# MoayedHajiAli/ElasticDiffusion-official

Measured on AMD Instinct MI355X. Metric: images/sec at 50 steps (SDXL 2048x1024), higher is better.
Workload: dtype fp16

## Files before the change

elasticdiffusion_official_amd/csrc/attention_kernels.hip:

```cpp
#include <hip/hip_runtime.h>
#include <stdint.h>

#include "elastic_hip.h"

namespace {

constexpr int D = 64;
constexpr int QB = 128;
constexpr int KT = 64;
constexpr int K_LD = 72;
constexpr int V_LD_TR = 96;
constexpr int V_LD_T = 68;

typedef float f32x16 __attribute__((ext_vector_type(16)));
typedef float f32x8 __attribute__((ext_vector_type(8)));
typedef short s16x4 __attribute__((ext_vector_type(4)));
typedef short s16x8 __attribute__((ext_vector_type(8)));
typedef __bf16 bf16x8 __attribute__((ext_vector_type(8)));
typedef _Float16 f16x8 __attribute__((ext_vector_type(8)));

struct alignas(16) Vec16 { uint32_t w[4]; };
struct alignas(8) Vec8 { uint32_t w[2]; };

struct BF {
// ... 174 lines not shown
#pragma unroll
      for (int kb = 0; kb < 2; ++kb)
#pragma unroll
        for (int r = 0; r < 16; ++r) {
          const float e = __builtin_amdgcn_exp2f(__builtin_fmaf(s[qn][kb][r], sl, -mb));
          s[qn][kb][r] = e;
          psum += e;
        }
      l_run[qn] = __builtin_fmaf(l_run[qn], alpha, psum);
#pragma unroll
      for (int i = 0; i < 16; ++i) {
        oacc[qn][0][i] *= alpha;
        oacc[qn][1][i] *= alpha;
      }
    }

#pragma unroll
    for (int st = 0; st < 4; ++st) {
      typename T::v8 pf[QN];
#pragma unroll
      for (int qn = 0; qn < QN; ++qn) {
        f32x8 pv;
#pragma unroll
        for (int j = 0; j < 8; ++j) pv[j] = s[qn][st >> 1][8 * (st & 1) + j];
        pf[qn] = T::pack(pv);
      }
#pragma unroll
      for (int db = 0; db < 2; ++db) {
        Vec16 vf;
        if (TR) {
          const int row = 16 * st + 4 * hi + ((lane & 15) >> 2);
          const int col = 32 * db + 16 * ((lane >> 4) & 1) + 4 * (lane & 3);
          typedef s16x4 __attribute__((address_space(3))) * lds_s16x4_ptr;
          const s16x4 lo = __builtin_amdgcn_ds_read_tr16_b64_v4i16((lds_s16x4_ptr)(&sm.v[buf][row * V_LD_TR + col]));
          const s16x4 hi4 = __builtin_amdgcn_ds_read_tr16_b64_v4i16((lds_s16x4_ptr)(&sm.v[buf][(row + 8) * V_LD_TR + col]));
          const s16x8 both = __builtin_shufflevector(lo, hi4, 0, 1, 2, 3, 4, 5, 6, 7);
          vf = __builtin_bit_cast(Vec16, both);
        } else {
          const uint16_t* vrow = &sm.v[buf][(32 * db + ln) * V_LD_T + 16 * st + 4 * hi];
          const Vec8 lo = *reinterpret_cast<const Vec8*>(vrow);
          const Vec8 hi8 = *reinterpret_cast<const Vec8*>(vrow + 8);
          vf.w[0] = lo.w[0], vf.w[1] = lo.w[1], vf.w[2] = hi8.w[0], vf.w[3] = hi8.w[1];
        }
#pragma unroll
        for (int qn = 0; qn < QN; ++qn) oacc[qn][db] = T::mfma(as_v8<typename T::v8>(vf), pf[qn], oacc[qn][db]);
      }
    }

    if (t + 1 < n_tiles) write_lds(buf ^ 1);
    __syncthreads();
  }

#pragma unroll
  for (int qn = 0; qn < QN; ++qn) {
    const float l_tot = l_run[qn] + __shfl_xor(l_run[qn], 32, 64);
    const float inv = 1.0f / l_tot;
    if (q_row[qn] < p.Nq) {
      uint16_t* orow = og + (int64_t)q_row[qn] * p.o_sn;
#pragma unroll
      for (int db = 0; db < 2; ++db)
#pragma unroll
        for (int g = 0; g < 4; ++g) {
          f32x8 tmp;
#pragma unroll
          for (int e = 0; e < 4; ++e) tmp[e] = oacc[qn][db][4 * g + e] * inv, tmp[4 + e] = 0.f;
          const Vec16 packed = __builtin_bit_cast(Vec16, T::pack(tmp));
          Vec8 out8 = {{packed.w[0], packed.w[1]}};
          *reinterpret_cast<Vec8*>(orow + 32 * db + 8 * g + 4 * hi) = out8;
        }
    }
  }
}


constexpr float RESCALE_LOG2 = 6.0f;
constexpr float RESCALE_SUM_MAX = 64.0f;

template <int NK>
struct SmemPipe {
  uint16_t k[NK][KT * K_LD];
  uint16_t v[3][KT * V_LD_TR];
};

template <typename T>
__device__ __forceinline__ void qk_tile(const uint16_t* kt, int ln, int hi, const typename T::v8 (&qf)[4], f32x16 (&s)[2]) {
#pragma unroll
  for (int i = 0; i < 16; ++i) s[0][i] = s[1][i] = 0.f;
#pragma unroll
  for (int ks = 0; ks < 4; ++ks)
#pragma unroll
    for (int kb = 0; kb < 2; ++kb) {
      const Vec16 kf = *reinterpret_cast<const Vec16*>(&kt[(32 * kb + ln) * K_LD + 16 * ks + 8 * hi]);
      s[kb] = T::mfma(as_v8<typename T::v8>(kf), qf[ks], s[kb]);
    }
}

__device__ __forceinline__ Vec16 v_frag_tr(const uint16_t* vt, int lane, int hi, int st, int db) {
  const int row = 16 * st + 4 * hi + ((lane & 15) >> 2);
  const int col = 32 * db + 16 * ((lane >> 4) & 1) + 4 * (lane & 3);
  typedef s16x4 __attribute__((address_space(3))) * lds_s16x4_ptr;
  const s16x4 lo = __builtin_amdgcn_ds_read_tr16_b64_v4i16((lds_s16x4_ptr)(&vt[row * V_LD_TR + col]));
  const s16x4 hi4 = __builtin_amdgcn_ds_read_tr16_b64_v4i16((lds_s16x4_ptr)(&vt[(row + 8) * V_LD_TR + col]));
  return __builtin_bit_cast(Vec16, __builtin_shufflevector(lo, hi4, 0, 1, 2, 3, 4, 5, 6, 7));
}

template <typename T>
__device__ __forceinline__ void pv_tile(const uint16_t* vt, int lane, int hi, const typename T::v8 (&pf)[4], f32x16 (&o)[2]) {
#pragma unroll
  for (int st = 0; st < 4; ++st)
#pragma unroll
    for (int db = 0; db < 2; ++db)
      o[db] = T::mfma(as_v8<typename T::v8>(v_frag_tr(vt, lane, hi, st, db)), pf[st], o[db]);
}

typedef __amdgpu_buffer_rsrc_t BufRsrc;
typedef uint32_t u32x4 __attribute__((ext_vector_type(4)));
__device__ __forceinline__ BufRsrc make_rsrc(const void* base, int64_t bytes) {
  const uint64_t a = (uint64_t)base;
  const uint32_t lo = __builtin_amdgcn_readfirstlane((int)(uint32_t)a), hi = __builtin_amdgcn_readfirstlane((int)(uint32_t)(a >> 32));
  const uint32_t n = __builtin_amdgcn_readfirstlane((int)(uint32_t)(bytes > 0xffffffffll ? 0xffffffffll : (bytes < 0 ? 0 : bytes)));
  return __builtin_amdgcn_make_buffer_rsrc((void*)(((uint64_t)hi << 32) | lo),  0, (int)n, 0x00020000);
}
__device__ __forceinline__ Vec16 buf_load16(BufRsrc rs, uint32_t voff, uint32_t soff) {
  const u32x4 v = __builtin_bit_cast(u32x4, __builtin_amdgcn_raw_buffer_load_b128(rs, voff, soff, 0));
  Vec16 o = {{v[0], v[1], v[2], v[3]}};
  return o;
}


template <typename T, int NDB = 2>
__device__ __forceinline__ void store_o_row(uint16_t* orow, const f32x16 (&o)[NDB], float inv, int hi, bool valid, int dh = 64) {
#pragma unroll
  for (int db = 0; db < NDB; ++db) {
    uint32_t part[4][2];
#pragma unroll
    for (int g = 0; g < 4; ++g) {
      f32x8 tmp;
#pragma unroll
      for (int e = 0; e < 4; ++e) tmp[e] = o[db][4 * g + e] * inv, tmp[4 + e] = 0.f;
      const Vec16 packed = __builtin_bit_cast(Vec16, T::pack(tmp));
      part[g][0] = packed.w[0], part[g][1] = packed.w[1];
    }
#pragma unroll
    for (int gp = 0; gp < 2; ++gp) {
      const int ge = 2 * gp, go = 2 * gp + 1;
      const uint32_t r0 = __shfl_xor(hi ? part[ge][0] : part[go][0], 32, 64);
      const uint32_t r1 = __shfl_xor(hi ? part[ge][1] : part[go][1], 32, 64);
      Vec16 out;
      if (hi) out = Vec16{{r0, r1, part[go][0], part[go][1]}};
      else out = Vec16{{part[ge][0], part[ge][1], r0, r1}};
      const int d0 = 32 * db + 8 * (hi ? go : ge);
      if (valid && d0 < dh) *reinterpret_cast<Vec16*>(orow + d0) = out;
    }
  }
}

struct True { static constexpr bool value = true; };
struct False { static constexpr bool value = false; };

struct SoftmaxRun {
  float mb;
  float l;
  float mx;
  float use;
  float alpha;
  float psum;
};

template <typename T>
__device__ __forceinline__ void softmax_slice(int i, f32x16 (&s)[2], float sl, SoftmaxRun& r, typename T::v8 (&pf)[4]) {
  if (i < 2) {
    float mx = (i == 0) ? -INFINITY : r.mx;
#pragma unroll
    for (int j = 0; j < 16; j += 2) mx = fmaxf(fmaxf(mx, s[i][j]), s[i][j + 1]);
    r.mx = mx;
    asm volatile("" : "+v"(r.mx));
  } else if (i == 2) {
    const float mx = fmaxf(r.mx, __shfl_xor(r.mx, 32, 64));
    const float mbn = mx * sl;
    r.use = (mbn - r.mb > RESCALE_LOG2) ? mbn : r.mb;
    r.alpha = __builtin_amdgcn_exp2f(r.mb - r.use);
    r.mb = r.use;
    r.psum = 0.f;
    asm volatile("" : "+v"(r.use), "+v"(r.alpha));
  } else if (i < 15) {
    const int g = (i - 3) / 3, w = (i - 3) % 3;
    const int f0 = 8 * g + 3 * w, n = (w == 2) ? 2 : 3;
#pragma unroll
    for (int j = 0; j < n; ++j) {
      const int f = f0 + j;
      const float e = __builtin_amdgcn_exp2f(__builtin_fmaf(s[f >> 4][f & 15], sl, -r.use));
      s[f >> 4][f & 15] = e;
      r.psum += e;
    }
    asm volatile("" : "+v"(r.psum));
    if (w == 2) {
      f32x8 pv;
#pragma unroll
      for (int j = 0; j < 8; ++j) pv[j] = s[g >> 1][8 * (g & 1) + j];
      pf[g] = T::pack(pv);
      asm volatile("" : "+v"(pf[g]));
    }
  } else {
    r.l = __builtin_fmaf(r.l, r.alpha, r.psum);
  }
}

template <typename T, bool EXP2>
__device__ __forceinline__ void softmax_slice_lazy(int i, f32x16 (&s)[2], float sl, SoftmaxRun& r, typename T::v8 (&pf)[4]) {
  if (i == 0) r.psum = 0.f;
#pragma unroll
  for (int j = 0; j < 2; ++j) {
    const int f = 2 * i + j;
    const float e = EXP2 ? __builtin_amdgcn_exp2f(s[f >> 4][f & 15])
                         : __builtin_amdgcn_exp2f(__builtin_fmaf(s[f >> 4][f & 15], sl, -r.mb));
    s[f >> 4][f & 15] = e;
    r.psum += e;
  }
  asm volatile("" : "+v"(r.psum));
  if ((i & 3) == 3) {
    const int g = i >> 2;
    f32x8 pv;
#pragma unroll
    for (int j = 0; j < 8; ++j) pv[j] = s[g >> 1][8 * (g & 1) + j];
    pf[g] = T::pack(pv);
    asm volatile("" : "+v"(pf[g]));
  }
}

template <typename T>
__device__ __forceinline__ void resoftmax_tile(const uint16_t* kt, int ln, int hi, const typename T::v8 (&qf)[4],
                                               f32x16 (&s)[2], float sl, SoftmaxRun& r, typename T::v8 (&pf)[4]) {
  qk_tile<T>(kt, ln, hi, qf, s);
  float mx = s[0][0];
#pragma unroll
  for (int j = 1; j < 16; ++j) mx = fmaxf(mx, s[0][j]);
#pragma unroll
  for (int j = 0; j < 16; ++j) mx = fmaxf(mx, s[1][j]);
  mx = fmaxf(mx, __shfl_xor(mx, 32, 64));
  const float use = fmaxf(r.mb, mx * sl);
  r.alpha = __builtin_amdgcn_exp2f(r.mb - use);
  r.mb = use;
  float psum = 0.f;
#pragma unroll
  for (int g = 0; g < 4; ++g) {
    f32x8 pv;
#pragma unroll
    for (int j = 0; j < 8; ++j) {
      const int f = 8 * g + j;
      pv[j] = __builtin_amdgcn_exp2f(__builtin_fmaf(s[f >> 4][f & 15], sl, -use));
      psum += pv[j];
    }
    pf[g] = T::pack(pv);
  }
  r.psum = psum;
}

template <typename T, bool HAS_PV, bool HAS_NEXT, bool LAZY, bool EXP2, int DEPTH, class Filler>
__device__ __forceinline__ void pipe_region(Filler&& filler, const uint16_t* k_next, const uint16_t* v_prev, int lane, int ln, int hi,
                                            const typename T::v8 (&qf)[4], f32x16 (&s_cur)[2], f32x16 (&s_next)[2],
                                            const typename T::v8 (&p_prev)[4], typename T::v8 (&p_cur)[4],
                                            f32x16 (&o)[2], float sl, SoftmaxRun& run, const f32x16& negm) {
  constexpr int NQK = HAS_NEXT ? 8 : 0, N = NQK + (HAS_PV ? 8 : 0);
  auto fetch = [&](int i) -> Vec16 {
    if (i < NQK) return *reinterpret_cast<const Vec16*>(&k_next[(32 * (i & 1) + ln) * K_LD + 16 * (i >> 1) + 8 * hi]);
    const int j = i - NQK;
    return v_frag_tr(v_prev, lane, hi, j >> 1, j & 1);
  };
  if (HAS_NEXT && !EXP2) {
#pragma unroll
    for (int i = 0; i < 16; ++i) s_next[0][i] = s_next[1][i] = 0.f;
  }
  Vec16 ring[DEPTH + 1];
#pragma unroll
  for (int r = 0; r <= DEPTH; ++r) ring[r] = Vec16{{0u, 0u, 0u, 0u}};
#pragma unroll
  for (int r = 0; r < DEPTH; ++r)
    if (r < N) ring[r] = fetch(r);
#pragma unroll
  for (int i = 0; i < 16; ++i) {
    if (i < N) {
      if (i + DEPTH < N) ring[(i + DEPTH) % (DEPTH + 1)] = fetch(i + DEPTH);
      const Vec16 a_cur = ring[i % (DEPTH + 1)];
      if (i < NQK) {
        if (EXP2 && i < 2) s_next[i & 1] = T::mfma(as_v8<typename T::v8>(a_cur), qf[0], negm);
        else s_next[i & 1] = T::mfma(as_v8<typename T::v8>(a_cur), qf[i >> 1], s_next[i & 1]);
        asm volatile("" : "+v"(s_next[i & 1]));
      } else {
        const int j = i - NQK;
        o[j & 1] = T::mfma(as_v8<typename T::v8>(a_cur), p_prev[j >> 1], o[j & 1]);
        asm volatile("" : "+v"(o[j & 1]));
      }
    }
    if (LAZY) softmax_slice_lazy<T, EXP2>(i, s_cur, sl, run, p_cur);
    else softmax_slice<T>(i, s_cur, sl, run, p_cur);
    filler(i);
    __builtin_amdgcn_sched_barrier(0);
  }
}

template <typename T, bool LAZY, bool EXP2 = false, int DEPTH = 1, int WAVES = 4>
__global__ void __launch_bounds__(64 * WAVES, 2)
k_flash_attn_pipe(const Params p) {
  static_assert(LAZY || !EXP2, "the exponent-domain variant is built on the lazy-maximum loop");
  static_assert(WAVES == 4 || WAVES == 8, "4 or 8 waves per workgroup");
  constexpr int NK = LAZY ? 3 : 2;
  constexpr int NST = 8 / WAVES;
  __shared__ SmemPipe<NK> sm;
  const int tid = threadIdx.x;
  const int lane = tid & 63, wave = tid >> 6;
  const int ln = lane & 31, hi = lane >> 5;
  int bh, qblk;
  {
    const int id = blockIdx.x, per = 8 * p.nqb, grp = id / per, r = id - grp * per;
    if ((grp + 1) * 8 <= p.BH) {
      bh = grp * 8 + (r & 7);
      qblk = r >> 3;
    } else {
      bh = grp * 8 + r / p.nqb;
      qblk = r % p.nqb;
    }
  }
  const int b = bh / p.H, h = bh - b * p.H;
  const uint16_t* qg = p.q + b * p.q_sb + h * D;
  const uint16_t* kg = p.k + b * p.k_sb + h * D;
  const uint16_t* vg = p.v + b * p.v_sb + h * D;
  uint16_t* og = p.o + b * p.o_sb + h * D;

  const int q_row = qblk * (32 * WAVES) + wave * 32 + ln;
  typename T::v8 qf[4];
#pragma unroll
  for (int ks = 0; ks < 4; ++ks) qf[ks] = as_v8<typename T::v8>(load_row16(qg, p.q_sn, q_row, p.Nq, 16 * ks + 8 * hi));

  const BufRsrc k_rs = make_rsrc(kg, ((int64_t)(p.Nk - 1) * p.k_sn + D) * 2);
  const BufRsrc v_rs = make_rsrc(vg, ((int64_t)(p.Nk - 1) * p.v_sn + D) * 2);
  const int st_row = tid >> 3, st_col = (tid & 7) * 8;
  const uint32_t k_off = (uint32_t)(((int64_t)st_row * p.k_sn + st_col) * 2), k_half = (uint32_t)(32 * p.k_sn * 2);
  const uint32_t v_off = (uint32_t)(((int64_t)st_row * p.v_sn + st_col) * 2), v_half = (uint32_t)(32 * p.v_sn * 2);
  Vec16 kreg[NST], vreg[NST];
  auto load_k = [&](int t) {
    const uint32_t base = k_off + (uint32_t)t * 2u * k_half;
#pragma unroll
    for (int i = 0; i < NST; ++i) kreg[i] = buf_load16(k_rs, base + i * k_half, 0);
  };
  auto load_v = [&](int t) {
    const uint32_t base = v_off + (uint32_t)t * 2u * v_half;
#pragma unroll
    for (int i = 0; i < NST; ++i) vreg[i] = buf_load16(v_rs, base + i * v_half, 0);
  };
  auto write_k = [&](int buf) {
// ... 75 lines not shown
    }
    const int tmp = vb_prev;
    vb_prev = vb_cur, vb_cur = vb_next, vb_next = tmp;
    const int ktmp = kb_cur;
    kb_cur = kb_next, kb_next = kb_write, kb_write = NK == 3 ? ktmp : kb_cur;
    __syncthreads();
  };

  if (n_full > 0) {
    qk_tile<T>(sm.k[0], ln, hi, qf, sA);
    if (EXP2) {
      float mx = sA[0][0];
#pragma unroll
      for (int j = 1; j < 16; ++j) mx = fmaxf(mx, sA[0][j]);
#pragma unroll
      for (int j = 0; j < 16; ++j) mx = fmaxf(mx, sA[1][j]);
      mx = fmaxf(mx, __shfl_xor(mx, 32, 64));
      run.mb = mx;
#pragma unroll
      for (int i = 0; i < 16; ++i) sA[0][i] -= mx, sA[1][i] -= mx, negm[i] = -mx;
      asm volatile("" : "+v"(negm));
    }
    __syncthreads();
    if (n_full == 1) {
      iter(False{}, False{}, 0, sA, sB, pB, pA);
    } else {
      iter(False{}, True{}, 0, sA, sB, pB, pA);
      int t = 1;
      for (; t + 2 < n_full; t += 2) {
        iter(True{}, True{}, t, sB, sA, pA, pB);
        iter(True{}, True{}, t + 1, sA, sB, pB, pA);
      }
      if (n_full - t == 2) {
        iter(True{}, True{}, t, sB, sA, pA, pB);
        iter(True{}, False{}, t + 1, sA, sB, pB, pA);
      } else {
        iter(True{}, False{}, t, sB, sA, pA, pB);
      }
    }
    if ((n_full - 1) & 1) pv_tile<T>(sm.v[vb_prev], lane, hi, pB, oacc);
    else pv_tile<T>(sm.v[vb_prev], lane, hi, pA, oacc);
  }

  if (n_tiles > n_full) {
    f32x16 s[2];
    qk_tile<T>(sm.k[kb_cur], ln, hi, qf, s);
#pragma unroll
    for (int kb = 0; kb < 2; ++kb)
#pragma unroll
      for (int r = 0; r < 16; ++r)
        if (n_full * KT + 32 * kb + 8 * (r >> 2) + 4 * hi + (r & 3) >= p.Nk) s[kb][r] = -INFINITY;
    float mx = s[0][0];
#pragma unroll
    for (int r = 1; r < 16; ++r) mx = fmaxf(mx, s[0][r]);
#pragma unroll
    for (int r = 0; r < 16; ++r) mx = fmaxf(mx, s[1][r]);
    mx = fmaxf(mx, __shfl_xor(mx, 32, 64));
    const float use = fmaxf(run.mb, mx * sl);
    const float alpha = __builtin_amdgcn_exp2f(run.mb - use);
    float psum = 0.f;
#pragma unroll
    for (int kb = 0; kb < 2; ++kb)
#pragma unroll
      for (int r = 0; r < 16; ++r) {
        const float e = __builtin_amdgcn_exp2f(__builtin_fmaf(s[kb][r], sl, -use));
        s[kb][r] = e;
        psum += e;
      }
    run.l = __builtin_fmaf(run.l, alpha, psum);
#pragma unroll
    for (int i = 0; i < 16; ++i) {
      oacc[0][i] *= alpha;
      oacc[1][i] *= alpha;
    }
    typename T::v8 pf[4];
#pragma unroll
    for (int st = 0; st < 4; ++st) {
      f32x8 pv;
#pragma unroll
      for (int j = 0; j < 8; ++j) pv[j] = s[st >> 1][8 * (st & 1) + j];
      pf[st] = T::pack(pv);
    }
    pv_tile<T>(sm.v[vb_cur], lane, hi, pf, oacc);
  }

  const float l_tot = run.l + __shfl_xor(run.l, 32, 64);
  const float inv = 1.0f / l_tot;
  store_o_row<T>(og + (int64_t)q_row * p.o_sn, oacc, inv, hi, q_row < p.Nq);
}

constexpr int SK_QBLOCKS = 4;

template <int NKB>
struct SmemSmall {
  uint16_t k[32 * NKB * K_LD];
  uint16_t v[32 * NKB * V_LD_TR];
};

template <typename T, int NKB>
__global__ void __launch_bounds__(256, 2)
k_flash_attn_smallkv(const Params p) {
  __shared__ SmemSmall<NKB> sm;
  const int tid = threadIdx.x;
  const int lane = tid & 63, wave = tid >> 6;
  const int ln = lane & 31, hi = lane >> 5;
  const int nqg = p.nqb;
  const int bh = blockIdx.x / nqg, qgrp = blockIdx.x - bh * nqg;
  const int b = bh / p.H, h = bh - b * p.H;
  const uint16_t* qg = p.q + b * p.q_sb + h * D;
  const uint16_t* kg = p.k + b * p.k_sb + h * D;
  const uint16_t* vg = p.v + b * p.v_sb + h * D;
  uint16_t* og = p.o + b * p.o_sb + h * D;

  for (int idx = tid; idx < 32 * NKB * 8; idx += 256) {
    const int row = idx >> 3, col = (idx & 7) * 8;
    *reinterpret_cast<Vec16*>(&sm.k[row * K_LD + col]) = load_row16(kg, p.k_sn, row, p.Nk, col);
    *reinterpret_cast<Vec16*>(&sm.v[row * V_LD_TR + col]) = load_row16(vg, p.v_sn, row, p.Nk, col);
  }
  __syncthreads();
  const float sl = p.scale_log2e;

  for (int qb = 0; qb < SK_QBLOCKS; ++qb) {
    const int q_row = (qgrp * SK_QBLOCKS + qb) * QB + wave * 32 + ln;
    if ((qgrp * SK_QBLOCKS + qb) * QB + wave * 32 >= p.Nq) break;
    typename T::v8 qf[4];
#pragma unroll
    for (int ks = 0; ks < 4; ++ks) qf[ks] = as_v8<typename T::v8>(load_row16(qg, p.q_sn, q_row, p.Nq, 16 * ks + 8 * hi));
    f32x16 s[NKB];
#pragma unroll
    for (int kb = 0; kb < NKB; ++kb)
#pragma unroll
      for (int i = 0; i < 16; ++i) s[kb][i] = 0.f;
#pragma unroll
    for (int ks = 0; ks < 4; ++ks)
#pragma unroll
      for (int kb = 0; kb < NKB; ++kb) {
        const Vec16 kf = *reinterpret_cast<const Vec16*>(&sm.k[(32 * kb + ln) * K_LD + 16 * ks + 8 * hi]);
        s[kb] = T::mfma(as_v8<typename T::v8>(kf), qf[ks], s[kb]);
      }
    float mx = -INFINITY;
#pragma unroll
    for (int kb = 0; kb < NKB; ++kb)
#pragma unroll
      for (int r = 0; r < 16; ++r) {
        if (32 * kb + 8 * (r >> 2) + 4 * hi + (r & 3) >= p.Nk) s[kb][r] = -INFINITY;
        mx = fmaxf(mx, s[kb][r]);
      }
    mx = fmaxf(mx, __shfl_xor(mx, 32, 64));
    const float mb = mx * sl;
    float psum = 0.f;
#pragma unroll
    for (int kb = 0; kb < NKB; ++kb)
#pragma unroll
      for (int r = 0; r < 16; ++r) {
        const float e = __builtin_amdgcn_exp2f(__builtin_fmaf(s[kb][r], sl, -mb));
        s[kb][r] = e;
        psum += e;
      }
    psum += __shfl_xor(psum, 32, 64);
    const float inv = 1.0f / psum;
    f32x16 o[2];
#pragma unroll
    for (int i = 0; i < 16; ++i) o[0][i] = o[1][i] = 0.f;
#pragma unroll
    for (int st = 0; st < 2 * NKB; ++st) {
      f32x8 pv;
// ... 128 lines not shown
#pragma unroll
    for (int r = 0; r < 16; ++r) mx = fmaxf(mx, s[1][r]);
    mx = fmaxf(mx, __shfl_xor(mx, 32, 64));
    const float m_new = fmaxf(m_run, mx);
    const float mb = m_new * sl;
    const float alpha = __builtin_amdgcn_exp2f(__builtin_fmaf(m_run, sl, -mb));
    m_run = m_new;
    float psum = 0.f;
#pragma unroll
    for (int kb = 0; kb < 2; ++kb)
#pragma unroll
      for (int r = 0; r < 16; ++r) {
        const float e = __builtin_amdgcn_exp2f(__builtin_fmaf(s[kb][r], sl, -mb));
        s[kb][r] = e;
        psum += e;
      }
    l_run = __builtin_fmaf(l_run, alpha, psum);
#pragma unroll
    for (int db = 0; db < G::NDB; ++db)
#pragma unroll
      for (int i = 0; i < 16; ++i) oacc[db][i] *= alpha;

#pragma unroll
    for (int st = 0; st < 4; ++st) {
      f32x8 pv;
#pragma unroll
      for (int j = 0; j < 8; ++j) pv[j] = s[st >> 1][8 * (st & 1) + j];
      const typename T::v8 pf = T::pack(pv);
#pragma unroll
      for (int db = 0; db < G::NDB; ++db) {
        const int row = 16 * st + 4 * hi + ((lane & 15) >> 2);
        const int col = 32 * db + 16 * ((lane >> 4) & 1) + 4 * (lane & 3);
        typedef s16x4 __attribute__((address_space(3))) * lds_s16x4_ptr;
        const s16x4 lo = __builtin_amdgcn_ds_read_tr16_b64_v4i16((lds_s16x4_ptr)(&sm.v[buf][row * G::VLD + col]));
        const s16x4 hi4 = __builtin_amdgcn_ds_read_tr16_b64_v4i16((lds_s16x4_ptr)(&sm.v[buf][(row + 8) * G::VLD + col]));
        const Vec16 vf = __builtin_bit_cast(Vec16, __builtin_shufflevector(lo, hi4, 0, 1, 2, 3, 4, 5, 6, 7));
        oacc[db] = T::mfma(as_v8<typename T::v8>(vf), pf, oacc[db]);
      }
    }
    if (t + 1 < n_tiles) write_lds(buf ^ 1);
    __syncthreads();
  }

  const float l_tot = l_run + __shfl_xor(l_run, 32, 64);
  const float inv = 1.0f / l_tot;
  store_o_row<T, G::NDB>(og + (int64_t)q_row * p.o_sn, oacc, inv, hi, q_row < p.Nq, DH);
}

}

extern "C" {

int ed_flash_attention(const void* q, const void* k, const void* v, void* out, int dtype, int B, int H, int Nq, int Nk,
                       int head_dim, int64_t q_sb, int64_t q_sn, int64_t k_sb, int64_t k_sn, int64_t v_sb, int64_t v_sn,
                       int64_t o_sb, int64_t o_sn, float scale, int v_path, void* stream) {
  if (B == 0 || H == 0 || Nq == 0) return 0;
  if (Nk <= 0) return (int)hipErrorInvalidValue;
  if (head_dim != D) {
    if (head_dim != 40 && head_dim != 80 && head_dim != 160) return (int)hipErrorInvalidValue;
    if (dtype != ED_BF16 && dtype != ED_F16) return (int)hipErrorInvalidValue;
    if ((((uintptr_t)q | (uintptr_t)k | (uintptr_t)v) & 15u) || ((uintptr_t)out & 7u)) return (int)hipErrorInvalidValue;
    if ((q_sb | q_sn | k_sb | k_sn | v_sb | v_sn) % 8 || (o_sb | o_sn) % 4) return (int)hipErrorInvalidValue;
    Params p;
    p.q = (const uint16_t*)q, p.k = (const uint16_t*)k, p.v = (const uint16_t*)v, p.o = (uint16_t*)out;
    p.Nq = Nq, p.Nk = Nk, p.H = H, p.BH = B * H, p.nqb = (Nq + QB - 1) / QB;
    p.q_sb = q_sb, p.q_sn = q_sn, p.k_sb = k_sb, p.k_sn = k_sn, p.v_sb = v_sb, p.v_sn = v_sn, p.o_sb = o_sb, p.o_sn = o_sn;
    p.scale_log2e = scale * 1.44269504088896340736f;
    const int64_t nb = (int64_t)p.BH * p.nqb;
    if (nb > 0x7fffffff) return (int)hipErrorInvalidValue;
    const dim3 grid((unsigned)nb), block(256);
    hipStream_t st = (hipStream_t)stream;
#define ED_FG(DHV)                                                                      \
  if (dtype == ED_BF16) k_flash_attn_gen<BF, DHV><<<grid, block, 0, st>>>(p);           \
  else k_flash_attn_gen<HF, DHV><<<grid, block, 0, st>>>(p);
    if (head_dim == 40) { ED_FG(40) } else if (head_dim == 80) { ED_FG(80) } else { ED_FG(160) }
#undef ED_FG
    return (int)hipGetLastError();
  }
  if ((((uintptr_t)q | (uintptr_t)k | (uintptr_t)v) & 15u) || ((uintptr_t)out & 7u)) return (int)hipErrorInvalidValue;
  if ((q_sb | q_sn | k_sb | k_sn | v_sb | v_sn) % 8 || (o_sb | o_sn) % 4) return (int)hipErrorInvalidValue;
  Params p;
  p.q = (const uint16_t*)q, p.k = (const uint16_t*)k, p.v = (const uint16_t*)v, p.o = (uint16_t*)out;
  hipStream_t st = (hipStream_t)stream;
  if ((v_path >= 4 && v_path <= 10)) {
    if (v_path == 8 && Nk > 160) return (int)hipErrorInvalidValue;
    if ((v_path == 6 || v_path == 7 || v_path == 9 || v_path == 10) && Nk < 64) return (int)hipErrorInvalidValue;
    if (v_path != 8 && ((int64_t)(Nk + 2 * KT) * (k_sn > v_sn ? k_sn : v_sn) * 2 >= 0x7fffffffll)) return (int)hipErrorInvalidValue;
    const int rows_per_wg = v_path == 8 ? QB * SK_QBLOCKS : (v_path >= 9 ? 2 * QB : QB);
    p.Nq = Nq, p.Nk = Nk, p.H = H, p.BH = B * H, p.nqb = (Nq + rows_per_wg - 1) / rows_per_wg;
    p.q_sb = q_sb, p.q_sn = q_sn, p.k_sb = k_sb, p.k_sn = k_sn, p.v_sb = v_sb, p.v_sn = v_sn, p.o_sb = o_sb, p.o_sn = o_sn;
    p.scale_log2e = scale * 1.44269504088896340736f;
    const int64_t nb = (int64_t)p.BH * p.nqb;
    if (nb > 0x7fffffff) return (int)hipErrorInvalidValue;
    const dim3 grid((unsigned)nb), block(256);
    if (dtype != ED_BF16 && dtype != ED_F16) return (int)hipErrorInvalidValue;
    if (v_path == 4) {
      if (dtype == ED_BF16) k_flash_attn_pipe<BF, false><<<grid, block, 0, st>>>(p);
      else k_flash_attn_pipe<HF, false><<<grid, block, 0, st>>>(p);
    } else if (v_path == 5) {
      if (dtype == ED_BF16) k_flash_attn_pipe<BF, true><<<grid, block, 0, st>>>(p);
      else k_flash_attn_pipe<HF, true><<<grid, block, 0, st>>>(p);
    } else if (v_path == 6) {
      if (dtype == ED_BF16) k_flash_attn_pipe<BF, true, true><<<grid, block, 0, st>>>(p);
      else k_flash_attn_pipe<HF, true, true><<<grid, block, 0, st>>>(p);
    } else if (v_path == 7) {
      if (dtype == ED_BF16) k_flash_attn_pipe<BF, false, false, 3><<<grid, block, 0, st>>>(p);
      else k_flash_attn_pipe<HF, false, false, 3><<<grid, block, 0, st>>>(p);
    } else if (v_path == 9) {
      if (dtype == ED_BF16) k_flash_attn_pipe<BF, false, false, 1, 8><<<grid, dim3(512), 0, st>>>(p);
      else k_flash_attn_pipe<HF, false, false, 1, 8><<<grid, dim3(512), 0, st>>>(p);
    } else if (v_path == 10) {
      if (dtype == ED_BF16) k_flash_attn_pipe<BF, true, false, 1, 8><<<grid, dim3(512), 0, st>>>(p);
      else k_flash_attn_pipe<HF, true, false, 1, 8><<<grid, dim3(512), 0, st>>>(p);
    } else if (Nk <= 64) {
      if (dtype == ED_BF16) k_flash_attn_smallkv<BF, 2><<<grid, block, 0, st>>>(p);
      else k_flash_attn_smallkv<HF, 2><<<grid, block, 0, st>>>(p);
    } else if (Nk <= 96) {
      if (dtype == ED_BF16) k_flash_attn_smallkv<BF, 3><<<grid, block, 0, st>>>(p);
      else k_flash_attn_smallkv<HF, 3><<<grid, block, 0, st>>>(p);
    } else {
      if (dtype == ED_BF16) k_flash_attn_smallkv<BF, 5><<<grid, block, 0, st>>>(p);
      else k_flash_attn_smallkv<HF, 5><<<grid, block, 0, st>>>(p);
    }
    return (int)hipGetLastError();
  }
  const int qn = (v_path & 2) ? 2 : 1;
  p.Nq = Nq, p.Nk = Nk, p.H = H, p.BH = B * H, p.nqb = (Nq + QB * qn - 1) / (QB * qn);
  p.q_sb = q_sb, p.q_sn = q_sn, p.k_sb = k_sb, p.k_sn = k_sn, p.v_sb = v_sb, p.v_sn = v_sn, p.o_sb = o_sb, p.o_sn = o_sn;
  p.scale_log2e = scale * 1.44269504088896340736f;
  const int64_t blocks = (int64_t)p.BH * p.nqb;
  if (blocks > 0x7fffffff) return (int)hipErrorInvalidValue;
  const dim3 grid((unsigned)blocks), block(256);
#define ED_FA(T)                                                                 \
  if (v_path == 0) k_flash_attn_fwd<T, true, 1><<<grid, block, 0, st>>>(p);      \
  else if (v_path == 1) k_flash_attn_fwd<T, false, 1><<<grid, block, 0, st>>>(p); \
  else if (v_path == 2) k_flash_attn_fwd<T, true, 2><<<grid, block, 0, st>>>(p);  \
  else if (v_path == 3) k_flash_attn_fwd<T, false, 2><<<grid, block, 0, st>>>(p); \
  else return (int)hipErrorInvalidValue;
  if (dtype == ED_BF16) {
    ED_FA(BF)
  } else if (dtype == ED_F16) {
    ED_FA(HF)
  } else {
    return (int)hipErrorInvalidValue;
  }
#undef ED_FA
  return (int)hipGetLastError();
}

}
```

elasticdiffusion_official_amd/ops.py:

```python
import torch

from . import _hip

ED_F32, ED_F16, ED_BF16 = 0, 1, 2
_DTYPE = {torch.float32: ED_F32, torch.float16: ED_F16, torch.bfloat16: ED_BF16}


_LAUNCH = {"device": None}


def _stream_of(t):
    if _LAUNCH["device"] is None:
        _LAUNCH["device"] = t.device
    return _stream()


def _stream():
    dev = _LAUNCH["device"]
    if dev is None:
        raise RuntimeError("internal: _stream() before any device tensor argument")
    return torch.cuda.current_stream(dev).cuda_stream


class KernelTimer:
# ... 903 lines not shown
    if not (isinstance(a, torch.Tensor) and a.is_cuda and a.dim() == 4 and a.dtype == torch.float16):
        _reject("conv3x3_f32out_s2: a must be an fp16 [B,C,H,W] tensor on the MI355X; no CPU fallback")
    B, C3, Hi, Wi = a.shape
    N = w.shape[0]
    cl = torch.channels_last
    if tuple(w.shape) != (N, C3, 3, 3) or w.dtype != torch.float16 or not conv3x3_f32out_s2_ok(B, Hi, Wi, C3, N):
        _reject(f"conv3x3_f32out_s2: unsupported shape a {tuple(a.shape)} w {tuple(w.shape)}")
    if not a.is_contiguous(memory_format=cl) or not w.is_contiguous(memory_format=cl):
        _reject("conv3x3_f32out_s2: a and w must be channels_last")
    H, W = Hi // 2, Wi // 2
    out = torch.empty((B, N, H, W), dtype=torch.float32, device=a.device, memory_format=cl)
    TIMER.note_work("ed_conv3x3_nhwc_f32out_s2", flops=2.0 * B * H * W * 9 * C3 * N, nbytes=2.0 * (B * Hi * Wi * C3 + 9 * C3 * N) + 4.0 * B * H * W * N)
    _call("ed_conv3x3_nhwc_f32out_s2", a.data_ptr(), w.data_ptr(), _opt(bias, torch.float32, "bias"), out.data_ptr(), _DTYPE[torch.float16],
          B, H, W, C3, N, float(out_scale), None if act_absmax is None else act_absmax.data_ptr(), _stream_of(a))
    return out


def softmax_rows_(x, scale=1.0):
    cols = x.shape[-1]
    if cols % 4 and x.numel() != cols:
        _reject("softmax_rows_: cols must be a multiple of 4")
    TIMER.note_work("ed_softmax_rows", nbytes=3.0 * x.numel() * 4)
    _call("ed_softmax_rows", _dev(x, torch.float32, "x"), x.numel() // cols, cols, float(scale), _stream())
    return x


VAE_ATTENTION_CHUNK_BYTES = 1 << 30


def vae_attention(q, k, v):
    B, N, C = q.shape
    scale = C ** -0.5
    rows = max(64, min(N, VAE_ATTENTION_CHUNK_BYTES // (4 * N * B) // 64 * 64)) if N > 256 else N
    kt = k.transpose(1, 2)
    if rows >= N:
        return torch.bmm(softmax_rows_(torch.bmm(q, kt), scale), v)
    out = torch.empty_like(q)
    for a in range(0, N, rows):
        s = torch.bmm(q[:, a:a + rows], kt)
        out[:, a:a + rows] = torch.bmm(softmax_rows_(s, scale), v)
    return out


FLASH_V_PATH = None
FLASH_HEAD_DIMS = (40, 64, 80, 160)
FLASH_EXP2 = False
_ENV_VARIANT = __import__("os").environ.get("ED_FLASH_VARIANT")
LOG2E = 1.4426950408889634


def _pipe_fits(Nk, row_stride):
    return Nk >= 128 and (Nk + 128) * row_stride * 2 < 2 ** 31


def flash_prescale(Nq, Nk, row_stride, scale=0.125):
    if FLASH_V_PATH is not None:
        want = int(FLASH_V_PATH)
    elif _ENV_VARIANT is not None:
        want = -1 if _ENV_VARIANT == "legacy" else int(_ENV_VARIANT)
    else:
        want = 6 if FLASH_EXP2 else -1
    return scale * LOG2E if (want == 6 and _pipe_fits(Nk, row_stride)) else None


def _flash_variant(B, heads, Nq, Nk, k=None, v=None, prescaled=False):
    fits = k is None or _pipe_fits(Nk, max(k.stride(1), v.stride(1)))
    if prescaled:
        if not (Nk >= 128 and fits):
            _reject("flash_attention: exponent-domain q needs the pipelined kernel (Nk >= 128, 32-bit K / V offsets)")
        return 6
    if FLASH_V_PATH is not None and int(FLASH_V_PATH) != 6:
        return int(FLASH_V_PATH)
    legacy = 2 if (Nq >= 2048 and Nk >= 1024 and B * heads * (Nq // 256) >= 1024) else 0
    if _ENV_VARIANT == "legacy":
        return legacy
    if _ENV_VARIANT is not None and int(_ENV_VARIANT) != 6:
        want = int(_ENV_VARIANT)
        if want in (4, 5, 7, 9, 10):
            return want if (Nk >= 128 and fits) else (8 if Nk <= 96 else legacy)
        return want if (want != 8 or Nk <= SMALLKV_MAX_KEYS) else legacy
    if Nk <= 96 or _stream_two_chunks(Nq, Nk):
        return 8
    if Nk >= 128 and fits:
        return FLASH_DEFAULT_PIPE
    return legacy


SMALLKV_MAX_KEYS = 160


def _stream_two_chunks(Nq, Nk):
    return 128 <= Nk <= SMALLKV_MAX_KEYS and Nq >= 4096


FLASH_DEFAULT_PIPE = 5


def flash_attention(q, k, v, heads, v_path=None, prescaled=False):
    B, Nq, HD = q.shape
    Nk = k.shape[1]
    hd = HD // heads
    if HD != heads * hd or hd not in FLASH_HEAD_DIMS or k.shape != (B, Nk, HD) or v.shape != (B, Nk, HD):
        _reject(f"flash_attention: head_dim must be one of {FLASH_HEAD_DIMS} and shapes consistent (q {tuple(q.shape)}, "
                f"k {tuple(k.shape)}, v {tuple(v.shape)}, heads {heads})")
    if hd != 64 and (prescaled or v_path is not None):
        _reject("flash_attention: kernel variants exist for head_dim 64 only")
    for t, name in ((q, "q"), (k, "k"), (v, "v")):
        if not t.is_cuda or t.dtype != q.dtype or t.stride(2) != 1:
            _reject(f"flash_attention: {name} must be a 16-bit tensor on the MI355X with unit last stride; no CPU fallback")
        if _LAUNCH["device"] is None:
            _LAUNCH["device"] = t.device
        elif _LAUNCH["device"] != t.device:
            _reject(f"flash_attention: {name} lives on {t.device}, q on {_LAUNCH['device']}")
    if v_path is not None and (int(v_path) == 6) != bool(prescaled):
        _reject("flash_attention: v_path 6 takes exponent-domain q (prescaled=True) and nothing else does")
    out = torch.empty(B, Nq, HD, dtype=q.dtype, device=q.device)
    TIMER.note_work("ed_flash_attention", flops=4.0 * B * heads * Nq * Nk * hd,
                    nbytes=2.0 * q.element_size() * HD * B * (Nq + Nk))
    variant = 0 if hd != 64 else (_flash_variant(B, heads, Nq, Nk, k, v, prescaled) if v_path is None else int(v_path))
    _call("ed_flash_attention", q.data_ptr(), k.data_ptr(), v.data_ptr(), out.data_ptr(), _code(q, "q"), B, heads, Nq, Nk,
          hd, q.stride(0), q.stride(1), k.stride(0), k.stride(1), v.stride(0), v.stride(1), out.stride(0), out.stride(1),
          hd ** -0.5, variant, _stream())
    return out


CANNY_MAX_DIM = 8192


def _canny_dims(t, name, channels):
    if t.dim() == 2 and 1 in channels:
        H, W, C = t.shape[0], t.shape[1], 1
    elif t.dim() == 3 and t.shape[2] in channels:
        H, W, C = t.shape
    else:
        _reject(f"{name} must be uint8 [H,W,C] with C in {sorted(channels)}{' or [H,W]' if 1 in channels else ''}, got {tuple(t.shape)}")
    if not (1 <= H <= CANNY_MAX_DIM and 1 <= W <= CANNY_MAX_DIM):
        _reject(f"{name}: H and W must be in 1..{CANNY_MAX_DIM}, got {H} x {W}")
    return H, W, C


def _canny_threshold(v, name):
    import math
    if not math.isfinite(v):
        _reject(f"canny: {name} threshold must be finite, got {v}")
    return max(-2 ** 31, min(2 ** 31 - 1, int(math.floor(v))))


def canny_map(img, low=100, high=200):
    p_img = _dev(img, torch.uint8, "img")
    H, W, C = _canny_dims(img, "img", (1, 3))
    lo, hi = _canny_threshold(low, "low"), _canny_threshold(high, "high")
    cmap = torch.empty((H, W), dtype=torch.uint8, device=img.device)
    TIMER.note_work("ed_canny_map", nbytes=float(H * W * (C + 1)))
    _call("ed_canny_map", p_img, H, W, C, lo, hi, _dev(cmap, torch.uint8, "map"), _stream())
    return cmap


def canny_hysteresis(cmap):
    import ctypes
    p_map = _dev(cmap, torch.uint8, "map")
    H, W, _ = _canny_dims(cmap, "map", (1,))
    if cmap.dim() != 2:
        _reject(f"map must be [H,W], got {tuple(cmap.shape)}")
    if torch.cuda.is_current_stream_capturing():
        _reject("canny_hysteresis reads a device flag between passes and cannot be captured into a graph")
    ws = torch.empty(_hip.lib().ed_canny_workspace(H, W, 1) // 4, dtype=torch.int32, device=cmap.device)
    passes = ctypes.c_int32(0)
    TIMER.note_work("ed_canny_hysteresis", nbytes=float(H * W))
    _call("ed_canny_hysteresis", p_map, H, W, _dev(ws, torch.int32, "workspace"), ctypes.addressof(passes), _stream())
    return cmap, int(passes.value)


def canny_edges(cmap, out="u8"):
    if out not in ("u8", "cond"):
        raise ValueError(f"out must be 'u8' or 'cond', got {out!r}")
    p_map = _dev(cmap, torch.uint8, "map")
    H, W, _ = _canny_dims(cmap, "map", (1,))
# ... 354 lines not shown
```

Before: 0.1036.

## Add DMA-to-LDS flash attention kernel with swizzled LDS layout for SDXL self-attention shapes

Adds a new flash attention kernel that loads K/V tiles straight from global memory into LDS with buffer_load ... lds. This bypasses the register round trip and the padded staging copies. LDS tiles use an unpadded XOR-swizzled layout to avoid bank conflicts, and the QK/PV fragment readers gain a swizzle-aware path. The dispatcher routes a fixed allowlist of self-attention shapes (B, Nk, heads) to this kernel. The inline-asm m0/waitcnt handling and the shape allowlist add fragility.

```diff
diff --git a/elasticdiffusion_official_amd/csrc/attention_kernels.hip b/elasticdiffusion_official_amd/csrc/attention_kernels.hip
--- a/elasticdiffusion_official_amd/csrc/attention_kernels.hip
+++ b/elasticdiffusion_official_amd/csrc/attention_kernels.hip
@@ -280,7 +280,19 @@
   uint16_t v[3][KT * V_LD_TR];
 };
 
-template <typename T>
+__device__ __forceinline__ constexpr int swz(int row) { return ((row & 2) << 1) | ((row >> 2) & 3); }
+__device__ __forceinline__ int swz_k_lane(int ln, int hi) { return ln * D + ((hi ^ swz(ln)) << 3); }
+__device__ __forceinline__ int swz_v_lane(int lane, int hi) {
+  const int row = 4 * hi + ((lane & 15) >> 2), col = 16 * ((lane >> 4) & 1) + 4 * (lane & 3);
+  return row * D + ((((col >> 3) ^ swz(row)) << 3) | (col & 7));
+}
+template <bool SWZ>
+__device__ __forceinline__ int k_elem(int kb, int ln, int ks, int hi) {
+  if constexpr (SWZ) return 32 * kb * D + (ln ^ (ks << 4));
+  else return (32 * kb + ln) * K_LD + 16 * ks + 8 * hi;
+}
+
+template <typename T, bool SWZ = false>
 __device__ __forceinline__ void qk_tile(const uint16_t* kt, int ln, int hi, const typename T::v8 (&qf)[4], f32x16 (&s)[2]) {
 #pragma unroll
   for (int i = 0; i < 16; ++i) s[0][i] = s[1][i] = 0.f;
@@ -288,27 +300,33 @@
   for (int ks = 0; ks < 4; ++ks)
 #pragma unroll
     for (int kb = 0; kb < 2; ++kb) {
-      const Vec16 kf = *reinterpret_cast<const Vec16*>(&kt[(32 * kb + ln) * K_LD + 16 * ks + 8 * hi]);
+      const Vec16 kf = *reinterpret_cast<const Vec16*>(&kt[k_elem<SWZ>(kb, ln, ks, hi)]);
       s[kb] = T::mfma(as_v8<typename T::v8>(kf), qf[ks], s[kb]);
     }
 }
 
+template <bool SWZ = false>
 __device__ __forceinline__ Vec16 v_frag_tr(const uint16_t* vt, int lane, int hi, int st, int db) {
+  typedef s16x4 __attribute__((address_space(3))) * lds_s16x4_ptr;
+  if constexpr (SWZ) {
+    const s16x4 lo = __builtin_amdgcn_ds_read_tr16_b64_v4i16((lds_s16x4_ptr)(&vt[16 * st * D + (lane ^ (db << 5))]));
+    const s16x4 hi4 = __builtin_amdgcn_ds_read_tr16_b64_v4i16((lds_s16x4_ptr)(&vt[(16 * st + 8) * D + (lane ^ (db << 5) ^ 16)]));
+    return __builtin_bit_cast(Vec16, __builtin_shufflevector(lo, hi4, 0, 1, 2, 3, 4, 5, 6, 7));
+  }
   const int row = 16 * st + 4 * hi + ((lane & 15) >> 2);
   const int col = 32 * db + 16 * ((lane >> 4) & 1) + 4 * (lane & 3);
-  typedef s16x4 __attribute__((address_space(3))) * lds_s16x4_ptr;
   const s16x4 lo = __builtin_amdgcn_ds_read_tr16_b64_v4i16((lds_s16x4_ptr)(&vt[row * V_LD_TR + col]));
   const s16x4 hi4 = __builtin_amdgcn_ds_read_tr16_b64_v4i16((lds_s16x4_ptr)(&vt[(row + 8) * V_LD_TR + col]));
   return __builtin_bit_cast(Vec16, __builtin_shufflevector(lo, hi4, 0, 1, 2, 3, 4, 5, 6, 7));
 }
 
-template <typename T>
+template <typename T, bool SWZ = false>
 __device__ __forceinline__ void pv_tile(const uint16_t* vt, int lane, int hi, const typename T::v8 (&pf)[4], f32x16 (&o)[2]) {
 #pragma unroll
   for (int st = 0; st < 4; ++st)
 #pragma unroll
     for (int db = 0; db < 2; ++db)
-      o[db] = T::mfma(as_v8<typename T::v8>(v_frag_tr(vt, lane, hi, st, db)), pf[st], o[db]);
+      o[db] = T::mfma(as_v8<typename T::v8>(v_frag_tr<SWZ>(vt, lane, hi, st, db)), pf[st], o[db]);
 }
 
 typedef __amdgpu_buffer_rsrc_t BufRsrc;
@@ -426,10 +444,10 @@
   }
 }
 
-template <typename T>
+template <typename T, bool SWZ = false>
 __device__ __forceinline__ void resoftmax_tile(const uint16_t* kt, int ln, int hi, const typename T::v8 (&qf)[4],
                                                f32x16 (&s)[2], float sl, SoftmaxRun& r, typename T::v8 (&pf)[4]) {
-  qk_tile<T>(kt, ln, hi, qf, s);
+  qk_tile<T, SWZ>(kt, ln, hi, qf, s);
   float mx = s[0][0];
 #pragma unroll
   for (int j = 1; j < 16; ++j) mx = fmaxf(mx, s[0][j]);
@@ -454,16 +472,16 @@
   r.psum = psum;
 }
 
-template <typename T, bool HAS_PV, bool HAS_NEXT, bool LAZY, bool EXP2, int DEPTH, class Filler>
+template <typename T, bool HAS_PV, bool HAS_NEXT, bool LAZY, bool EXP2, int DEPTH, bool SWZ = false, class Filler>
 __device__ __forceinline__ void pipe_region(Filler&& filler, const uint16_t* k_next, const uint16_t* v_prev, int lane, int ln, int hi,
                                             const typename T::v8 (&qf)[4], f32x16 (&s_cur)[2], f32x16 (&s_next)[2],
                                             const typename T::v8 (&p_prev)[4], typename T::v8 (&p_cur)[4],
                                             f32x16 (&o)[2], float sl, SoftmaxRun& run, const f32x16& negm) {
   constexpr int NQK = HAS_NEXT ? 8 : 0, N = NQK + (HAS_PV ? 8 : 0);
   auto fetch = [&](int i) -> Vec16 {
-    if (i < NQK) return *reinterpret_cast<const Vec16*>(&k_next[(32 * (i & 1) + ln) * K_LD + 16 * (i >> 1) + 8 * hi]);
+    if (i < NQK) return *reinterpret_cast<const Vec16*>(&k_next[k_elem<SWZ>(i & 1, ln, i >> 1, hi)]);
     const int j = i - NQK;
-    return v_frag_tr(v_prev, lane, hi, j >> 1, j & 1);
+    return v_frag_tr<SWZ>(v_prev, lane, hi, j >> 1, j & 1);
   };
   if (HAS_NEXT && !EXP2) {
 #pragma unroll
@@ -705,6 +723,221 @@
       pf[st] = T::pack(pv);
     }
     pv_tile<T>(sm.v[vb_cur], lane, hi, pf, oacc);
+  }
+
+  const float l_tot = run.l + __shfl_xor(run.l, 32, 64);
+  const float inv = 1.0f / l_tot;
+  store_o_row<T>(og + (int64_t)q_row * p.o_sn, oacc, inv, hi, q_row < p.Nq);
+}
+
+#define ED_ATT_WAIT_VM(n) asm volatile("s_waitcnt vmcnt(" #n ")" ::: "memory")
+#define ED_ATT_BARRIER()                      \
+  do {                                        \
+    asm volatile("s_barrier" ::: "memory");   \
+    __builtin_amdgcn_sched_barrier(0);        \
+  } while (0)
+typedef __attribute__((address_space(3))) void* lds_ptr_t;
+
+__device__ __forceinline__ u32x4 make_rsrc_words(const void* base, int64_t bytes) {
+  const uint64_t a = (uint64_t)base;
+  u32x4 w;
+  w[0] = __builtin_amdgcn_readfirstlane((int)(uint32_t)a);
+  w[1] = __builtin_amdgcn_readfirstlane((int)((uint32_t)(a >> 32) & 0xffffu));
+  w[2] = __builtin_amdgcn_readfirstlane((int)(uint32_t)(bytes > 0xffffffffll ? 0xffffffffll : (bytes < 0 ? 0 : bytes)));
+  w[3] = 0x00020000u;
+  return w;
+}
+__device__ __forceinline__ void dma16(u32x4 rs, uint32_t lds_addr, uint32_t voff) {
+  asm volatile("s_mov_b32 m0, %0\n\ts_nop 0\n\tbuffer_load_dwordx4 %1, %2, 0 offen lds" ::"s"(lds_addr), "v"(voff), "s"(rs) : "memory");
+}
+
+struct SmemDma {
+  uint16_t k[3][KT * D];
+  uint16_t v[3][KT * D];
+};
+
+template <typename T, int OCC>
+__global__ void __launch_bounds__(256, OCC)
+k_flash_attn_dma(const Params p) {
+  __shared__ SmemDma sm;
+  const int tid = threadIdx.x;
+  const int lane = tid & 63, wave = __builtin_amdgcn_readfirstlane(tid >> 6);
+  const int ln = lane & 31, hi = lane >> 5;
+  int bh, qblk;
+  {
+    const int id = blockIdx.x, per = 8 * p.nqb, grp = id / per, r = id - grp * per;
+    if ((grp + 1) * 8 <= p.BH) {
+      bh = grp * 8 + (r & 7);
+      qblk = r >> 3;
+    } else {
+      bh = grp * 8 + r / p.nqb;
+      qblk = r % p.nqb;
+    }
+  }
+  const int b = bh / p.H, h = bh - b * p.H;
+  const uint16_t* qg = p.q + b * p.q_sb + h * D;
+  const uint16_t* kg = p.k + b * p.k_sb + h * D;
+  const uint16_t* vg = p.v + b * p.v_sb + h * D;
+  uint16_t* og = p.o + b * p.o_sb + h * D;
+
+  int xk = swz_k_lane(ln, hi), xv = swz_v_lane(lane, hi);
+  asm volatile("" : "+v"(xk), "+v"(xv));
+
+  const int q_row = qblk * QB + wave * 32 + ln;
+  typename T::v8 qf[4];
+#pragma unroll
+  for (int ks = 0; ks < 4; ++ks) qf[ks] = as_v8<typename T::v8>(load_row16(qg, p.q_sn, q_row, p.Nq, 16 * ks + 8 * hi));
+
+  const u32x4 k_rs = make_rsrc_words(kg, ((int64_t)(p.Nk - 1) * p.k_sn + D) * 2);
+  const u32x4 v_rs = make_rsrc_words(vg, ((int64_t)(p.Nk - 1) * p.v_sn + D) * 2);
+  const int st_row = tid >> 3, st_col = (((tid & 7) ^ swz(st_row)) << 3);
+  const uint32_t k_off = (uint32_t)(((int64_t)st_row * p.k_sn + st_col) * 2), k_half = (uint32_t)(32 * p.k_sn * 2);
+  const uint32_t v_off = (uint32_t)(((int64_t)st_row * p.v_sn + st_col) * 2), v_half = (uint32_t)(32 * p.v_sn * 2);
+  auto dma = [&](const u32x4 rs, uint16_t* tile, uint32_t off, uint32_t half, int i) {
+    dma16(rs, (uint32_t)(uintptr_t)(lds_ptr_t)(tile + (32 * i + 8 * wave) * D), off + i * half);
+  };
+
+  f32x16 oacc[2];
+  SoftmaxRun run;
+  run.mb = -INFINITY, run.l = 0.f, run.mx = 0.f, run.use = 0.f, run.alpha = 1.f, run.psum = 0.f;
+  const float sl = p.scale_log2e;
+  const int n_tiles = (p.Nk + KT - 1) / KT, n_full = p.Nk / KT;
+  f32x16 negm;
+#pragma unroll
+  for (int i = 0; i < 16; ++i) negm[i] = 0.f;
+
+  asm volatile("s_nop 4" ::: "memory");
+#pragma unroll
+  for (int i = 0; i < 2; ++i) dma(k_rs, sm.k[0], k_off, k_half, i);
+#pragma unroll
+  for (int i = 0; i < 2; ++i) dma(v_rs, sm.v[0], v_off, v_half, i);
+#pragma unroll
+  for (int i = 0; i < 2; ++i) dma(k_rs, sm.k[1], k_off + 2u * k_half, k_half, i);
+  ED_ATT_WAIT_VM(0);
+  ED_ATT_BARRIER();
+
+  f32x16 sA[2], sB[2];
+  typename T::v8 pA[4], pB[4];
+  int vb_prev = 2, vb_cur = 0, vb_next = 1;
+  int kb_cur = 0, kb_next = 1, kb_write = 2;
+  uint32_t k_run = k_off + 4u * k_half, v_run = v_off + 2u * v_half;
+
+  auto iter = [&](auto has_pv, auto has_next, int t, f32x16 (&s_cur)[2], f32x16 (&s_next)[2],
+                  typename T::v8 (&p_prev)[4], typename T::v8 (&p_cur)[4]) {
+    uint16_t* const kdst = sm.k[kb_write];
+    uint16_t* const vdst = sm.v[vb_next];
+    auto filler = [&](int i) {
+      if (i < 2) dma(k_rs, kdst, k_run, k_half, i);
+      else if (i < 4) dma(v_rs, vdst, v_run, v_half, i - 2);
+    };
+    int xk_t = xk, xv_t = xv;
+    asm volatile("" : "+v"(xk_t), "+v"(xv_t));
+    constexpr bool lazy = decltype(has_pv)::value;
+    pipe_region<T, decltype(has_pv)::value, decltype(has_next)::value, lazy, false, 1, true>(filler, sm.k[kb_next], sm.v[vb_prev], xv_t, xk_t,
+                                                                                             hi, qf, s_cur, s_next, p_prev, p_cur,
+                                                                                             oacc, sl, run, negm);
+    k_run += 2u * k_half, v_run += 2u * v_half;
+    asm volatile("" : "+v"(k_run), "+v"(v_run));
+    if (lazy) {
+      run.alpha = 1.0f;
+      if (__any(!(run.psum <= RESCALE_SUM_MAX))) {
+        int xk_s = xk;
+        asm volatile("" : "+v"(xk_s));
+        resoftmax_tile<T, true>(sm.k[kb_cur], xk_s, hi, qf, s_cur, sl, run, p_cur);
+      }
+      run.l = __builtin_fmaf(run.l, run.alpha, run.psum);
+    }
+    if (decltype(has_pv)::value && __any(run.alpha != 1.0f)) {
+#pragma unroll
+      for (int i = 0; i < 16; ++i) {
+        oacc[0][i] *= run.alpha;
+        oacc[1][i] *= run.alpha;
+      }
+    }
+    const int tmp = vb_prev;
+    vb_prev = vb_cur, vb_cur = vb_next, vb_next = tmp;
+    const int ktmp = kb_cur;
+    kb_cur = kb_next, kb_next = kb_write, kb_write = ktmp;
+    ED_ATT_WAIT_VM(2);
+    ED_ATT_BARRIER();
+  };
+
+  auto zero_o = [&]() {
+#pragma unroll
+    for (int i = 0; i < 16; ++i) oacc[0][i] = oacc[1][i] = 0.f;
+  };
+  if (n_full == 0) zero_o();
+  if (n_full > 0) {
+    int xk_0 = xk;
+    if (n_full == 1) {
+      asm volatile("" : "+v"(xk_0));
+      qk_tile<T, true>(sm.k[0], xk_0, hi, qf, sA);
+      iter(False{}, False{}, 0, sA, sB, pB, pA);
+      zero_o();
+      pv_tile<T, true>(sm.v[vb_prev], xv, hi, pA, oacc);
+    } else {
+      asm volatile("" : "+v"(xk_0));
+      qk_tile<T, true>(sm.k[0], xk_0, hi, qf, sA);
+      iter(False{}, True{}, 0, sA, sB, pB, pA);
+      zero_o();
+      int t = 1;
+      for (; t + 2 < n_full; t += 2) {
+        iter(True{}, True{}, t, sB, sA, pA, pB);
+        iter(True{}, True{}, t + 1, sA, sB, pB, pA);
+      }
+      if (n_full - t == 2) {
+        iter(True{}, True{}, t, sB, sA, pA, pB);
+        iter(True{}, False{}, t + 1, sA, sB, pB, pA);
+        pv_tile<T, true>(sm.v[vb_prev], xv, hi, pA, oacc);
+      } else {
+        iter(True{}, False{}, t, sB, sA, pA, pB);
+        pv_tile<T, true>(sm.v[vb_prev], xv, hi, pB, oacc);
+      }
+    }
+  }
+  ED_ATT_WAIT_VM(0);
+
+  if (n_tiles > n_full) {
+    ED_ATT_BARRIER();
+    f32x16 s[2];
+    qk_tile<T, true>(sm.k[kb_cur], xk, hi, qf, s);
+#pragma unroll
+    for (int kb = 0; kb < 2; ++kb)
+#pragma unroll
+      for (int r = 0; r < 16; ++r)
+        if (n_full * KT + 32 * kb + 8 * (r >> 2) + 4 * hi + (r & 3) >= p.Nk) s[kb][r] = -INFINITY;
+    float mx = s[0][0];
+#pragma unroll
+    for (int r = 1; r < 16; ++r) mx = fmaxf(mx, s[0][r]);
+#pragma unroll
+    for (int r = 0; r < 16; ++r) mx = fmaxf(mx, s[1][r]);
+    mx = fmaxf(mx, __shfl_xor(mx, 32, 64));
+    const float use = fmaxf(run.mb, mx * sl);
+    const float alpha = __builtin_amdgcn_exp2f(run.mb - use);
+    float psum = 0.f;
+#pragma unroll
+    for (int kb = 0; kb < 2; ++kb)
+#pragma unroll
+      for (int r = 0; r < 16; ++r) {
+        const float e = __builtin_amdgcn_exp2f(__builtin_fmaf(s[kb][r], sl, -use));
+        s[kb][r] = e;
+        psum += e;
+      }
+    run.l = __builtin_fmaf(run.l, alpha, psum);
+#pragma unroll
+    for (int i = 0; i < 16; ++i) {
+      oacc[0][i] *= alpha;
+      oacc[1][i] *= alpha;
+    }
+    typename T::v8 pf[4];
+#pragma unroll
+    for (int st = 0; st < 4; ++st) {
+      f32x8 pv;
+#pragma unroll
+      for (int j = 0; j < 8; ++j) pv[j] = s[st >> 1][8 * (st & 1) + j];
+      pf[st] = T::pack(pv);
+    }
+    pv_tile<T, true>(sm.v[vb_cur], xv, hi, pf, oacc);
   }
 
   const float l_tot = run.l + __shfl_xor(run.l, 32, 64);
@@ -999,11 +1232,11 @@
   Params p;
   p.q = (const uint16_t*)q, p.k = (const uint16_t*)k, p.v = (const uint16_t*)v, p.o = (uint16_t*)out;
   hipStream_t st = (hipStream_t)stream;
-  if ((v_path >= 4 && v_path <= 10)) {
+  if ((v_path >= 4 && v_path <= 12)) {
     if (v_path == 8 && Nk > 160) return (int)hipErrorInvalidValue;
     if ((v_path == 6 || v_path == 7 || v_path == 9 || v_path == 10) && Nk < 64) return (int)hipErrorInvalidValue;
     if (v_path != 8 && ((int64_t)(Nk + 2 * KT) * (k_sn > v_sn ? k_sn : v_sn) * 2 >= 0x7fffffffll)) return (int)hipErrorInvalidValue;
-    const int rows_per_wg = v_path == 8 ? QB * SK_QBLOCKS : (v_path >= 9 ? 2 * QB : QB);
+    const int rows_per_wg = v_path == 8 ? QB * SK_QBLOCKS : (v_path == 9 || v_path == 10 ? 2 * QB : QB);
     p.Nq = Nq, p.Nk = Nk, p.H = H, p.BH = B * H, p.nqb = (Nq + rows_per_wg - 1) / rows_per_wg;
     p.q_sb = q_sb, p.q_sn = q_sn, p.k_sb = k_sb, p.k_sn = k_sn, p.v_sb = v_sb, p.v_sn = v_sn, p.o_sb = o_sb, p.o_sn = o_sn;
     p.scale_log2e = scale * 1.44269504088896340736f;
@@ -1029,6 +1262,11 @@
     } else if (v_path == 10) {
       if (dtype == ED_BF16) k_flash_attn_pipe<BF, true, false, 1, 8><<<grid, dim3(512), 0, st>>>(p);
       else k_flash_attn_pipe<HF, true, false, 1, 8><<<grid, dim3(512), 0, st>>>(p);
+    } else if (v_path == 11) {
+      return (int)hipErrorInvalidValue;
+    } else if (v_path == 12) {
+      if (dtype == ED_BF16) k_flash_attn_dma<BF, 2><<<grid, block, 0, st>>>(p);
+      else k_flash_attn_dma<HF, 2><<<grid, block, 0, st>>>(p);
     } else if (Nk <= 64) {
       if (dtype == ED_BF16) k_flash_attn_smallkv<BF, 2><<<grid, block, 0, st>>>(p);
       else k_flash_attn_smallkv<HF, 2><<<grid, block, 0, st>>>(p);
diff --git a/elasticdiffusion_official_amd/ops.py b/elasticdiffusion_official_amd/ops.py
--- a/elasticdiffusion_official_amd/ops.py
+++ b/elasticdiffusion_official_amd/ops.py
@@ -1009,7 +1009,7 @@
     if Nk <= 96 or _stream_two_chunks(Nq, Nk):
         return 8
     if Nk >= 128 and fits:
-        return FLASH_DEFAULT_PIPE
+        return FLASH_DMA_PIPE if (Nq == Nk and (B, Nk, heads) in FLASH_DMA_SHAPES) else FLASH_DEFAULT_PIPE
     return legacy
 
 
@@ -1020,6 +1020,8 @@
     return 128 <= Nk <= SMALLKV_MAX_KEYS and Nq >= 4096
 
 
+FLASH_DMA_PIPE = 12
+FLASH_DMA_SHAPES = frozenset({(40, 4096, 10), (40, 1024, 20), (12, 4096, 10), (12, 1024, 20)})
 FLASH_DEFAULT_PIPE = 5
 
 
```

Result: no change. 0.1043, median of 6 (+0.7%).
